# at-wat/mcl_3dl

Hardware: AMD Instinct MI355X
Metric: particle·point evals/sec; filter-update Hz @ 4096 particles × 16k-pt scan (higher is better)
Workload: dtype f32

## Files before the change

### mcl_3dl_amd/csrc/host_map_compilers.h

```cpp
#pragma once

namespace
{
int build_lik_grid(mcl3dl_hip_ctx* ctx);
int build_dda_grid(mcl3dl_hip_ctx* ctx);
int ensure_map_dev(mcl3dl_hip_ctx* ctx);
int cloud_minmax(mcl3dl_hip_ctx* ctx, const float4* pts, long long n, float* host6, unsigned long long* host_cnt);

void kd_ray_radii(const mcl3dl_hip_ctx* ctx, float* grid_min, float* r1, float* r2)
{
  const float mn = std::min({ ctx->map_grid[0], ctx->map_grid[1], ctx->map_grid[2] });
  const float mx = std::max({ ctx->map_grid[0], ctx->map_grid[1], ctx->map_grid[2] });
  *grid_min = mn;
  *r1 = static_cast<float>(std::sqrt(2.0) * mx / 2.0);
  *r2 = static_cast<float>(mn * 2 + std::sqrt(2.0) * mx / 2.0);
}

bool lik_cell_is_beams(const mcl3dl_hip_ctx* ctx)
{
  return !ctx->lik_params_set && ctx->beam_raycast == 1;
}

float lik_cell_edge(const mcl3dl_hip_ctx* ctx)
{
// ... 611 lines not shown
    g.brick_table = table;
    g.rec = ctx->cand_rec.as<float4>();
    g.ovf = ctx->cand_ovf.as<float4>();
    g.ox = cp.ox;
    g.oy = cp.oy;
    g.oz = cp.oz;
    g.inv_ex = cp.inv_ex;
    g.inv_ey = cp.inv_ey;
    g.inv_ez = cp.inv_ez;
    g.nvx = cp.nvx;
    g.nvy = cp.nvy;
    g.nvz = cp.nvz;
    g.nbx = cp.nbx;
    g.nby = cp.nby;
    g.nbz = cp.nbz;
    g.mul24_ok = (static_cast<long long>(cp.nbx) * cp.nby < (1ll << 24) && cp.nbz < (1 << 24)) ? 1 : 0;
    g.off32_ok = (rec_bytes * static_cast<unsigned long long>(n_vox) < (1ull << 32)) ? 1 : 0;
    g.rec_bytes32 = bytes32(rec_bytes * static_cast<unsigned long long>(n_vox));
    g.rec_parts = static_cast<int>(cap);
    set_word_format(g, co.packed, ctx->match_dist_min);
    ctx->cand_parts = cap;
    g.ovf_bytes32 = bytes32(64ull * (n_ovf ? n_ovf : 1));
    g.ti_empty = static_cast<uint32_t>(n_table);
    ctx->footprint[5] = sizeof(int) * n_table;
    ctx->footprint[6] = rec_bytes * static_cast<size_t>(n_vox);
    ctx->footprint[7] = 64ull * n_ovf;
    ctx->cand_stats[0] = n_bricks;
    ctx->cand_stats[1] = static_cast<double>(total);
    ctx->cand_stats[2] = static_cast<double>(kept);
    ctx->cand_stats[3] = ms2;
    ctx->cand_stats[4] = static_cast<double>(co.hist3[0]);
    ctx->cand_stats[5] = static_cast<double>(co.hist3[1]);
    ctx->cand_over8 = static_cast<double>(co.hist3[2]);
    ctx->cand_stats[6] = n_ovf;
    ctx->cand_stats[7] = cp.ex / static_cast<double>(ctx->match_dist_min);
    ctx->cand_edge_ratio[0] = cp.ex / static_cast<double>(ctx->match_dist_min);
    ctx->cand_edge_ratio[1] = cp.ey / static_cast<double>(ctx->match_dist_min);
    ctx->cand_edge_ratio[2] = cp.ez / static_cast<double>(ctx->match_dist_min);
    ctx->cand_dirty = false;
    return 0;
  }
  return ctx->fail(-3, "the candidate index is built for lik_index = 2 only");
}

int build_cand_grid_budgeted(mcl3dl_hip_ctx* ctx, double ratio, uint32_t cap, double* ratio_used = nullptr)
{
// ... 111 lines not shown
  hipLaunchKernelGGL(mc_ovf_counts, dim3(static_cast<unsigned>((n_vox + 1 + 255) / 256)), dim3(256), 0, ctx->stream,
                     ctx->cand_rec.as<float4>(), n_vox, cap, ctx->rg.packed, ctx->rg.count_shift, ctx->rg.count_is_records, cnt);
  TRY(device_exclusive_scan(ctx, cnt, n_vox + 1));
  uint32_t live = 0;
  TRY(d2h(ctx, &live, cnt + n_vox, sizeof(uint32_t)));
  TRY(sync_stream(ctx));
  void* fresh = nullptr;
  const size_t cap_bytes = 64ull * (static_cast<size_t>(live) + live / 2 + 1024);
  HIP_TRY(hipMalloc(&fresh, cap_bytes));
  hipLaunchKernelGGL(mc_ovf_move, dim3(static_cast<unsigned>((n_vox + 255) / 256)), dim3(256), 0, ctx->stream,
                     ctx->cand_rec.as<float4>(), n_vox, cap, ctx->rg.packed, ctx->rg.count_shift, ctx->rg.ext_bits, ctx->rg.count_is_records, cnt,
                     ctx->cand_ovf.as<float4>(),
                     static_cast<float4*>(fresh));
  HIP_TRY(hipGetLastError());
  TRY(sync_stream(ctx));
  if (ctx->cand_ovf.p)
    HIP_TRY(hipFree(ctx->cand_ovf.p));
  ctx->cand_ovf.p = fresh;
  ctx->cand_ovf.cap = cap_bytes;
  ctx->cand_n_ovf = live;
  ctx->cand_ovf_leaked = 0;
  ctx->rg.ovf = ctx->cand_ovf.as<float4>();
  ctx->rg.ovf_bytes32 = bytes32(64ull * (live ? live : 1));
  ctx->footprint[7] = 64ull * live;
  ctx->cand_stats[6] = live;
  ++ctx->cand_ovf_compactions;
  return 0;
}

int update_cand_grid(mcl3dl_hip_ctx* ctx, size_t n_base, const std::vector<float4>& old_update, double* stats5)
{
  const size_t n_total = ctx->map_xyz.size() / 3;
  if (stats5)
    for (int i = 0; i < 6; ++i)
      stats5[i] = 0;
  if (ctx->cand_dirty || ctx->opt.lik_index != 2 || ctx->cand_n_points != n_base + old_update.size())
  {
    if (stats5)
      stats5[5] = ctx->cand_dirty ? 1 : ctx->opt.lik_index != 2 ? 2 : 3;
    ctx->cand_dirty = true;
    return 0;
  }
  CompileParams cp = ctx->cand_cp;
  const long long n_table = ctx->cand_n_table;
  std::vector<float4> fresh;
  TRY(rescaled_points(ctx, n_base, n_total - n_base, fresh, nullptr, nullptr));
// ... 123 lines not shown
  HIP_TRY(hipMemsetAsync(d_orphan.p, 0, sizeof(unsigned long long), ctx->stream));
  hipLaunchKernelGGL(mc_install_records, dim3(static_cast<unsigned>((n_sub_vox + 255) / 256)), dim3(256), 0, ctx->stream,
                     static_cast<const float4*>(d_subrec.p), static_cast<const int*>(d_sub_main.p), ovf_base, n_bricks_old,
                     n_sub_vox, ctx->cand_rec.as<float4>(), static_cast<unsigned long long*>(d_orphan.p), cap, ctx->rg.packed,
                     ctx->rg.count_shift, ctx->rg.count_is_records);
  HIP_TRY(hipGetLastError());
  unsigned long long orphaned = 0;
  TRY(d2h(ctx, &orphaned, d_orphan.p, sizeof(orphaned)));
  HIP_TRY(hipEventRecord(ev1, ctx->stream));
  TRY(sync_stream(ctx));
  float ms = 0.f;
  HIP_TRY(hipEventSynchronize(ev1));
  HIP_TRY(hipEventElapsedTime(&ms, ev0, ev1));
  ctx->cand_n_bricks = n_bricks;
  ctx->cand_n_ovf = ovf_base + co.n_ovf;
  ctx->cand_ovf_leaked += static_cast<uint32_t>(orphaned);
  ctx->cand_n_points = n_total;
  ctx->rg.brick_table = ctx->cand_table.as<int>();
  ctx->rg.rec = ctx->cand_rec.as<float4>();
  ctx->rg.ovf = ctx->cand_ovf.as<float4>();
  ctx->rg.off32_ok = (rec_bytes * 512 * n_bricks < (1ull << 32)) ? 1 : 0;
  ctx->rg.rec_bytes32 = bytes32(rec_bytes * 512 * n_bricks);
  ctx->rg.ovf_bytes32 = bytes32(64ull * (ctx->cand_n_ovf ? ctx->cand_n_ovf : 1));
  ctx->footprint[6] = rec_bytes * 512 * n_bricks;
  ctx->footprint[7] = 64ull * ctx->cand_n_ovf;
  ctx->cand_stats[0] = n_bricks;
  ctx->cand_stats[6] = ctx->cand_n_ovf;
  if (stats5)
  {
    stats5[0] = n_dirty;
    stats5[1] = n_new;
    stats5[2] = n_rel;
    stats5[3] = ms;
    stats5[4] = co.n_ovf;
  }
  return 0;
}

}
```

### mcl_3dl_amd/csrc/host_measure.h

```cpp
#pragma once
#include <type_traits>

namespace
{
int ensure_structures(mcl3dl_hip_ctx* ctx, bool need_lik, bool need_dda, bool need_cells = false)
{
  if (!ctx->has_map)
    return ctx->fail(-5, "no map: call mcl3dl_hip_set_map first");
  bool built = false;
  if (need_lik && ctx->opt.lik_index == 0 && !need_cells && !ctx->lik_params_set && (ctx->lik_cell_from_beam || lik_cell_is_beams(ctx)))
  {
    ctx->lik_params_set = true;
    if (ctx->lik_cell_from_beam)
      ctx->lik_dirty = ctx->lik_base_dirty = true;
  }
  if (need_lik && (ctx->opt.lik_index == 0 || need_cells) && ctx->lik_dirty)
  {
    TRY(build_lik_grid(ctx));
    built = true;
  }
  if (need_lik && ctx->opt.lik_index >= 1 && !need_cells && ctx->cand_dirty)
  {
    TRY(build_cand_grid(ctx));
    built = true;
// ... 211 lines not shown
  long long grid = 0;
};

Interleave interleave(long long n_beam, long long n_other)
{
  Interleave il;
  if (n_beam >= n_other)
    il.beam8 = static_cast<uint32_t>(std::min<long long>(8, (n_beam + n_other / 2) / n_other));
  else
    il.other8 = static_cast<uint32_t>(std::min<long long>(8, (n_other + n_beam / 2) / n_beam));
  const long long rounds = std::max((n_beam + 8 * il.beam8 - 1) / (8 * il.beam8), (n_other + 8 * il.other8 - 1) / (8 * il.other8));
  il.grid = rounds * 8 * (il.beam8 + il.other8);
  return il;
}

bool lik_defer_active(const mcl3dl_hip_ctx* ctx)
{
  if (ctx->opt.lik_defer == 0 || ctx->opt.lik_index != 2 || !ctx->rg.packed || ctx->rg.rec_parts != 4)
    return false;
  if (ctx->opt.lik_defer == 1)
    return true;
  const double with_cand = ctx->cand_stats[4], over4 = ctx->cand_stats[5];
  return with_cand > 0 && over4 / with_cand > LIK_DEFER_MIN_FRAC;
}

int ensure_chain(mcl3dl_hip_ctx* ctx, size_t n_p, int n_tiles, uint32_t* tag0)
{
  if (!ctx->chain_err)
  {
    volatile unsigned* w = ctx->zero_copy_supported ? static_cast<volatile unsigned*>(pinned_alloc(ctx, 64)) : nullptr;
    if (!w || !ctx->zero_copy_supported)
      return ctx->fail(-2, "strict_order = 3 needs page-locked memory the device can write in place");
    *w = 0u;
    ctx->chain_err = w;
  }
  const size_t need = sizeof(unsigned long long) * 2 * n_p;
  const bool fresh = need > ctx->chain_carry.cap;
  TRY(ensure(ctx, ctx->chain_carry, need));
  if (fresh || ctx->chain_tag > 0xffffffffu - static_cast<uint32_t>(n_tiles) - 2u)
  {
    HIP_TRY(hipMemsetAsync(ctx->chain_carry.p, 0, ctx->chain_carry.cap, ctx->stream));
    ctx->chain_tag = 1u;
  }
  *tag0 = ctx->chain_tag;
  ctx->chain_tag += static_cast<uint32_t>(n_tiles) + 1u;
  return 0;
// ... 365 lines not shown
    {
      const auto kernel = ctx->dg.ov_n > 0 ? beam_kernel<false, true> : beam_kernel<false, false>;
      hipLaunchKernelGGL(kernel, grid, dim3(256), 0, bs, c.d_pose, ctx->scan_beam.as<float4>(), static_cast<int>(ctx->n_b),
                         ctx->origins.as<float4>(), pl.n_rays, ctx->dg, beam_params(ctx), ctx->penalty.as<unsigned>(),
                         static_cast<RayStats*>(nullptr), prepared, static_cast<int>(ctx->n_o));
    }
    finish_beam(c, bs);
  }
  TRY(timing_end(ctx, ep, bs));
  if (overlap)
    HIP_TRY(hipEventRecord(ctx->ev_join, bs));
  HIP_TRY(hipGetLastError());
  return 0;
}

template <class Args>
Interleave merged_args(const MeasureCall& c, long long n_beam, long long n_other, Args* a)
{
  mcl3dl_hip_ctx* ctx = c.ctx;
  const Interleave il = interleave(n_beam, n_other);
  a->pose7 = c.d_pose;
  a->n_p = c.np;
  a->g = ctx->lg;
  a->rg = ctx->rg;
  a->prm = c.lp;
  a->scan_beam = ctx->scan_beam.as<float4>();
  a->n_b = static_cast<int>(ctx->n_b);
  a->origins = ctx->origins.as<float4>();
  a->n_rays = c.plan.n_rays;
  a->dg = ctx->dg;
  a->bp = beam_params(ctx);
  a->penalty = ctx->penalty.as<unsigned>();
  a->prepared = c.plan.prepared ? ctx->beam_origin.as<BeamOrigin>() : nullptr;
  a->n_o = static_cast<int>(ctx->n_o);
  a->beam8 = il.beam8;
  a->n_beam_blocks = static_cast<uint32_t>(n_beam);
  return il;
}

template <bool CHAIN>
void launch_lik_beam(const MeasureCall& c, long long t_blocks, const float4* scan, int n_s, int n_tiles, LikBeamArgs& a)
{
  mcl3dl_hip_ctx* ctx = c.ctx;
  const Interleave il = merged_args(c, c.plan.beam_blocks, t_blocks, &a);
  a.n_groups = c.plan.n_groups;
  a.strict_skew4 = STRICT_SKEW4;
  a.tiled8 = il.other8;
// ... 39 lines not shown
}

void launch_tiled(const MeasureCall& c, const float4* t_scan, int t_ns, int t_tiles, double* t_psum, unsigned* t_pcnt,
                  const uint32_t* t_perm, float* t_terms)
{
  mcl3dl_hip_ctx* ctx = c.ctx;
  const MeasurePlan& pl = c.plan;
  const long long t_blocks = tiled_blocks(t_tiles, pl.n_groups);
  if (pl.beam == BeamRoute::MergedTiled)
  {
    LikBeamArgs a{};
    a.partial_sum = t_psum;
    a.partial_cnt = t_pcnt;
    a.scan_perm = t_perm;
    a.strict_terms = t_terms;
    launch_lik_beam<false>(c, t_blocks, t_scan, t_ns, t_tiles, a);
    return;
  }
  dispatch_int<4, 8, 32, 16>(pl.group_size, [&](auto g) {
    dispatch_form(pl, [&](auto mode, auto coop, auto defer) {
      constexpr int G = decltype(g)::value;
      constexpr int MINW = G == 32 ? 4 : 8;
      hipLaunchKernelGGL((likelihood_tiled_kernel<G, decltype(mode)::value, MINW, decltype(coop)::value, decltype(defer)::value>), dim3(static_cast<unsigned>(t_blocks)),
                         dim3(256), 0, ctx->stream, c.d_pose, c.np, t_scan, t_ns, t_tiles, pl.n_groups, ctx->lg, ctx->rg, c.lp,
                         t_psum, t_pcnt, t_perm, t_terms, STRICT_SKEW4);
    });
  });
}

template <int GG>
void launch_strict_sum(mcl3dl_hip_ctx* ctx, const float* strict_terms, int ns, int np, int n_groups, float* d_lik, hipStream_t on,
                       int accumulate)
{
  constexpr int MAX_GPW = 64 / GG >= 4 ? 4 : (64 / GG >= 2 ? 2 : 1);
  int gpw = n_groups <= ctx->n_cus ? 1 : (n_groups <= 2 * ctx->n_cus ? 2 : 4);
  gpw = std::min(gpw, MAX_GPW);
  const auto launch = [&](auto chunk, auto per_wg) {
    constexpr int GPW = decltype(per_wg)::value;
    hipLaunchKernelGGL((lik_strict_sum_rows_kernel<GG, decltype(chunk)::value, GPW>), dim3((n_groups + GPW - 1) / GPW), dim3(1024),
                       0, on, strict_terms, ns, np, n_groups, d_lik, STRICT_SKEW4, accumulate);
  };
  using std::integral_constant;
  if constexpr (MAX_GPW >= 4)
    if (gpw == 4)
      return launch(integral_constant<int, 16384>{}, integral_constant<int, 4>{});
  if constexpr (MAX_GPW >= 2)
    if (gpw >= 2)
      return launch(integral_constant<int, 32768>{}, integral_constant<int, 2>{});
// ... 79 lines not shown
    hipEvent_t ev;
    hipStream_t st;
    ~ChainDone()
    {
      (void)hipEventRecord(ev, st);
    }
  } chain_done{ cs.ev, ctx->stream };
  float* const lik_out = c.d_lik ? c.d_lik : ctx->chain_lik.as<float>();
  const LikChain lc{ ctx->chain_carry.as<unsigned long long>(), pl.chain_tag0, lik_out, c.d_ratio, c.beam_ones(), ctx->chain_err };
  const dim3 grid(static_cast<unsigned>(pl.blocks));
  if (pl.lik == LikRoute::ChainMulti)
    hipLaunchKernelGGL((likelihood_chain_multi_kernel<4, 4>), grid, dim3(256), 0, ctx->stream, c.d_pose, c.np, c.scan, c.ns,
                       pl.n_tiles, pl.n_super, pl.n_groups, ctx->rg, c.lp, lc);
  else if (pl.beam == BeamRoute::MergedChain)
  {
    LikBeamArgs a{};
    a.ch = lc;
    launch_lik_beam<true>(c, pl.blocks, c.scan, c.ns, pl.n_tiles, a);
  }
  else
    dispatch_int<4, 8, 16>(pl.group_size, [&](auto g) {
      dispatch_form(pl, [&](auto mode, auto coop, auto defer) {
        hipLaunchKernelGGL((likelihood_tiled_kernel<decltype(g)::value, decltype(mode)::value, 8, decltype(coop)::value, decltype(defer)::value, true>),
                           grid, dim3(256), 0, ctx->stream, c.d_pose, c.np, c.scan, c.ns, pl.n_tiles, pl.n_groups, ctx->lg, ctx->rg, c.lp,
                           static_cast<double*>(nullptr), static_cast<unsigned*>(nullptr), static_cast<const uint32_t*>(nullptr),
                           static_cast<float*>(nullptr), 0, lc);
      });
    });
  return 0;
}

void launch_particle(const MeasureCall& c)
{
  mcl3dl_hip_ctx* ctx = c.ctx;
  const MeasurePlan& pl = c.plan;
  const uint32_t* row_perm = pl.rows ? ctx->scan_perm.as<uint32_t>() : nullptr;
  const size_t row_bytes = pl.rows ? sizeof(float) * static_cast<size_t>(chain_row_floats(c.ns)) : 0;
  if (pl.beam == BeamRoute::MergedParticle)
  {
    LikParticleBeamArgs a{};
    const Interleave il = merged_args(c, (pl.n_rays + pl.block - 1) / pl.block, c.np, &a);
    a.scan = c.scan;
    a.n_s = c.ns;
    a.out_lik = c.d_lik;
    a.out_ratio = c.d_ratio;
    a.coop = pl.coop ? 1 : 0;
    a.perm = row_perm;
// ... 198 lines not shown
```

### mcl_3dl_amd/csrc/host_options.h

```cpp
#pragma once

#include <cstdio>
#include <cstdlib>
#include <cstring>
#include <limits>

constexpr long long OVERLAP_MIN_RAYS = 262144;
constexpr int LIK_WIDE_MAX_PARTICLES = 512;
constexpr int PF_FUSED_MAX_PARTICLES = 1024;
constexpr int STRICT_ROWS_MAX_PARTICLES = 2048;
constexpr double POLL_QUERY_US = 5000.0;
constexpr double LIK_DEFER_MIN_FRAC = 0.03;
constexpr long long BEAM_PREPARE_MIN_RAYS = 32768;
constexpr int CHAIN_MULTI_MAX = 1536;

struct Options
{
  int overlap_models = 1;
  int lik_index = 2;
  int lik_small = 1;
  int lik_tiled = 1;
  int lik_tiled_min = 1024;
  int lik_group = 0;
  int lik_coop = 1;
  int pf_fused = 1;
  int strict_order = 2;
  int strict_auto_min = 28147;
  int strict_exact_max = 4096;
  double strict_auto_max_bytes = 0.0;
  int strict_chunk = 0;
  int scan_presorted = 0;
  int update_small = 1;
  int update_small_max = 512;
  int update_small_conformant = 0;
  int update_stage = 1;
  int update_zero_copy = 1;
  int poll_sync = 2;
  double poll_spin_us = 2000.0;
  bool test_late_structures = false;
  int cand_prune_coop = 1;
  int batch_slice = 0;
  double cand_voxel_ratio = 0.0;
  double cand_phase = 0.5;
  int cand_aniso = 2;
  double cand_aniso_max = 8.0;
  double index_budget_opt = -1.0;
  int cand_record_parts = 0;
// ... 197 lines not shown
```

### mcl_3dl_amd/csrc/likelihood_kernels.h

```cpp
#pragma once
#include <hip/hip_runtime.h>
#include <stdint.h>

#include "device_math.h"
#include "float_chain.h"
#include "map_structs.h"
#pragma clang fp contract(off)

namespace mcl3dl
{
template <bool STATS>
__device__ inline float nearest_d2(const LikGrid& g, float qx, float qy, float qz, unsigned& n_tested)
{
  const float fx = floorf((qx - g.ox) * g.inv_cell);
  const float fy = floorf((qy - g.oy) * g.inv_cell);
  const float fz = floorf((qz - g.oz) * g.inv_cell);
  float best = 3.0e38f;
  if (!(fx >= 1.0f && fy >= 1.0f && fz >= 1.0f && fx <= static_cast<float>(g.nx - 2) &&
        fy <= static_cast<float>(g.ny - 2) && fz <= static_cast<float>(g.nz - 2)))
    return best;
  const int cx = static_cast<int>(fx), cy = static_cast<int>(fy), cz = static_cast<int>(fz);
  uint32_t rs[9], re[9];
#pragma unroll
  for (int r = 0; r < 9; ++r)
// ... 68 lines not shown
            const float d2 = d2_simple(qx, qy, qz, p.x, p.y, p.z);
            const int idx = static_cast<int>(__float_as_uint(p.w));
            if (d2 < best || (d2 == best && best_idx >= 0 && idx < best_idx))
            {
              best = d2;
              best_idx = idx;
            }
          }
        }
  }
  out_index[i] = best_idx;
  if (out_sqdist)
    out_sqdist[i] = best_idx >= 0 ? best : -1.0f;
}


__device__ inline int floor_to_int(float x)
{
  int r;
  asm("v_cvt_flr_i32_f32 %0, %1" : "=v"(r) : "v"(x));
  return r;
}

__device__ inline bool rec_locate(const RecGrid& g, float qx, float qy, float qz, uint32_t& ti, uint32_t& sub)
{
  const int vx = floor_to_int((qx - g.ox) * g.inv_ex);
  const int vy = floor_to_int((qy - g.oy) * g.inv_ey);
  const int vz = floor_to_int((qz - g.oz) * g.inv_ez);
  if (g.mul24_ok)
    ti = __umul24(static_cast<uint32_t>(vz >> 3), static_cast<uint32_t>(g.nbx * g.nby)) +
         __umul24(static_cast<uint32_t>(vy >> 3), static_cast<uint32_t>(g.nbx)) + static_cast<uint32_t>(vx >> 3);
  else
    ti = (static_cast<uint32_t>(vz >> 3) * static_cast<uint32_t>(g.nby) + static_cast<uint32_t>(vy >> 3)) *
             static_cast<uint32_t>(g.nbx) + static_cast<uint32_t>(vx >> 3);
  sub = ((((static_cast<uint32_t>(vz) & 7u) << 3) | (static_cast<uint32_t>(vy) & 7u)) << 3) | (static_cast<uint32_t>(vx) & 7u);
  return static_cast<unsigned>(vx) < static_cast<unsigned>(g.nvx) && static_cast<unsigned>(vy) < static_cast<unsigned>(g.nvy) &&
         static_cast<unsigned>(vz) < static_cast<unsigned>(g.nvz);
}

__device__ inline float rec_overflow_min(const RecGrid& g, float qx, float qy, float qz, uint32_t n_records, uint32_t ext,
                                         float best)
{
  const float4* o = g.ovf + 4 * static_cast<size_t>(ext);
  for (uint32_t j = 0; j < 4u * n_records; ++j)
  {
    const float4 c = o[j];
    const float d = d2_simple(qx, qy, qz, c.x, c.y, c.z);
    best = d < best ? d : best;
  }
  return best;
}

// ... 53 lines not shown
  return __int_as_float(__builtin_amdgcn_update_dpp(0, __float_as_int(v), CTRL, 0xf, 0xf, true));
}
template <int CTRL>
__device__ inline uint32_t quad_u(uint32_t v)
{
  return static_cast<uint32_t>(__builtin_amdgcn_update_dpp(0, static_cast<int>(v), CTRL, 0xf, 0xf, true));
}
constexpr int QUAD_BCAST0 = 0x00, QUAD_BCAST1 = 0x55, QUAD_BCAST2 = 0xAA, QUAD_BCAST3 = 0xFF;
constexpr int QUAD_XOR1 = 0xB1, QUAD_XOR2 = 0x4E;

typedef unsigned int u32x4 __attribute__((ext_vector_type(4)));
__device__ inline float4 buffer_load_f4(__amdgpu_buffer_rsrc_t rs, uint32_t byte_offset)
{
  const u32x4 v = __builtin_amdgcn_raw_buffer_load_b128(rs, static_cast<int>(byte_offset), 0, 0);
  return make_float4(__uint_as_float(v.x), __uint_as_float(v.y), __uint_as_float(v.z), __uint_as_float(v.w));
}

__device__ inline unsigned long long lanes_gt_u32(uint32_t a, uint32_t b)
{
  return __builtin_amdgcn_uicmp(a, b, 34 );
}
constexpr unsigned long long QUAD_LANE0_MASK = 0x1111111111111111ull;

__device__ inline float quad_round(const float4* recs, uint32_t bytes32, uint32_t rec_index, float qx, float qy, float qz,
                                   int j, uint32_t (&w)[4])
{
  float4 R0, R1, R2, R3;
  if (bytes32)
  {
    const __amdgpu_buffer_rsrc_t rs =
        __builtin_amdgcn_make_buffer_rsrc(const_cast<float4*>(recs), 0, static_cast<int>(bytes32), 0x00020000);
    const uint32_t mine = rec_index << 6, part = static_cast<uint32_t>(j) << 4;
    R0 = buffer_load_f4(rs, quad_u<QUAD_BCAST0>(mine) + part);
    R1 = buffer_load_f4(rs, quad_u<QUAD_BCAST1>(mine) + part);
    R2 = buffer_load_f4(rs, quad_u<QUAD_BCAST2>(mine) + part);
    R3 = buffer_load_f4(rs, quad_u<QUAD_BCAST3>(mine) + part);
  }
  else
  {
    const float4* part = recs + j;
    R0 = part[4 * static_cast<size_t>(quad_u<QUAD_BCAST0>(rec_index))];
    R1 = part[4 * static_cast<size_t>(quad_u<QUAD_BCAST1>(rec_index))];
    R2 = part[4 * static_cast<size_t>(quad_u<QUAD_BCAST2>(rec_index))];
    R3 = part[4 * static_cast<size_t>(quad_u<QUAD_BCAST3>(rec_index))];
  }
  const float d0 = d2_simple(quad_f<QUAD_BCAST0>(qx), quad_f<QUAD_BCAST0>(qy), quad_f<QUAD_BCAST0>(qz), R0.x, R0.y, R0.z);
  const float d1 = d2_simple(quad_f<QUAD_BCAST1>(qx), quad_f<QUAD_BCAST1>(qy), quad_f<QUAD_BCAST1>(qz), R1.x, R1.y, R1.z);
  const float d2 = d2_simple(quad_f<QUAD_BCAST2>(qx), quad_f<QUAD_BCAST2>(qy), quad_f<QUAD_BCAST2>(qz), R2.x, R2.y, R2.z);
  const float d3 = d2_simple(quad_f<QUAD_BCAST3>(qx), quad_f<QUAD_BCAST3>(qy), quad_f<QUAD_BCAST3>(qz), R3.x, R3.y, R3.z);
  const bool odd = (j & 1) != 0, high = (j & 2) != 0;
  const uint32_t u0 = __float_as_uint(d0), u1 = __float_as_uint(d1), u2 = __float_as_uint(d2), u3 = __float_as_uint(d3);
  const uint32_t m01 = min(odd ? u1 : u0, quad_u<QUAD_XOR1>(odd ? u0 : u1));
  const uint32_t m23 = min(odd ? u3 : u2, quad_u<QUAD_XOR1>(odd ? u2 : u3));
  w[0] = __float_as_uint(R0.w);
  w[1] = __float_as_uint(R1.w);
  w[2] = __float_as_uint(R2.w);
  w[3] = __float_as_uint(R3.w);
  return __uint_as_float(min(high ? m23 : m01, quad_u<QUAD_XOR2>(high ? m01 : m23)));
}
// ... 375 lines not shown
  {
    if (out_lik)
      out_lik[p] = lik;
    if (out_ratio)
      out_ratio[p] = static_cast<float>(num) / static_cast<float>(n_s);
  }
}

struct LikChain
{
  unsigned long long* carry;
  uint32_t tag0;
  float* out_lik;
  float* out_ratio;
  float* also_fill;
  volatile unsigned* err;
};

__device__ inline unsigned long long chain_pack(uint32_t value, uint32_t tag)
{
  return (static_cast<unsigned long long>(tag) << 32) | value;
}

constexpr int CHAIN_POLL_MAX = 1 << 20;
constexpr int DEFER_QCAP = 96;

struct DeferQueue
{
  uint32_t word[4][DEFER_QCAP];
  uint16_t who[4][DEFER_QCAP];
};

__device__ inline float eval_coop_first(const RecGrid& rg, const LikParams& prm, const Vec3f pos, const Quat rot, const float4 v,
                                        bool have_point, int lane, bool& matched, bool& over, float& best, uint32_t& mine,
                                        unsigned long long& over_m)
{
  const Vec3f tp = vadd(qrot_trim(rot, Vec3f{ v.x, v.y, v.z }), pos);
  const float qx = tp.x * prm.wx, qy = tp.y * prm.wy, qz = tp.z * prm.wz;
  uint32_t ti, sub;
  const bool inside = rec_locate(rg, qx, qy, qz, ti, sub) && have_point;
  const int b = rg.brick_table[inside ? ti : rg.ti_empty];
  const bool valid = b >= 0;
  float dist = -1.0f;
  over = false;
  over_m = 0ull;
  best = 0.0f;
  mine = 0u;
  const unsigned long long valid_m = __builtin_amdgcn_ballot_w64(valid);
  if (valid_m != 0ull)
  {
    const uint32_t rec = (static_cast<uint32_t>(b) << 9) | sub;
    const uint32_t vrec = rg.rec_bytes32 ? rec : (valid ? rec : 0u);
    uint32_t w[4];
    best = quad_round(rg.rec, rg.rec_bytes32, vrec, qx, qy, qz, lane & 3, w);
    mine = own_word(w, lane & 3);
    over_m = valid_m & lanes_gt_u32(mine, rg.over_thr);
    if (rg.bound_step > 0.0f && over_m != 0ull)
    {
      asm volatile("");
      over_m &= __builtin_amdgcn_fcmpf(best, rec_bound2(rg, mine), 2 );
    }
    over = __builtin_amdgcn_inverse_ballot_w64(over_m);
    if (valid && !over && best < prm.r2)
    {
      const float s = sqrt_in_radius(best);
      dist = lik_dist(prm, s);
    }
  }
  matched = !(dist < 0.0f);
  return lik_term(prm, dist, matched);
}

template <int G, int LD>
__device__ inline void defer_drain(const RecGrid& rg, const LikParams& prm, const float (&s_pose)[G][8], float (&s_term)[G][LD],
                                   unsigned (&s_cnt)[G][4], const DeferQueue& q, int wave, int lane, uint32_t base, uint32_t n,
                                   const float4 v)
{
  const bool act = static_cast<uint32_t>(lane) < n;
  const uint32_t slot = act ? base + static_cast<uint32_t>(lane) : base;
  const uint32_t word = q.word[wave][slot];
  const uint32_t who = q.who[wave][slot];
  const int src = static_cast<int>(who & 63u), k = static_cast<int>(who >> 6);
  const Vec3f pt = { __shfl(v.x, src), __shfl(v.y, src), __shfl(v.z, src) };
  const Vec3f pos = { s_pose[k][0], s_pose[k][1], s_pose[k][2] };
  const Quat rot = { s_pose[k][3], s_pose[k][4], s_pose[k][5], s_pose[k][6] };
  const Vec3f tp = vadd(qrot_trim(rot, pt), pos);
  const float qx = tp.x * prm.wx, qy = tp.y * prm.wy, qz = tp.z * prm.wz;
  const int t_src = wave * 64 + src;
  float best = s_term[k][t_src];
  const uint32_t ext = word & rec_ext_mask(rg);
  const uint32_t rounds = act ? rec_overflow_records(word >> rg.count_shift, 4u, rg.count_is_records) : 0u;
  for (uint32_t r = 0; wave_any(r < rounds); ++r)
  {
    const bool more = r < rounds;
    uint32_t unused[4];
    const float m = quad_round(rg.ovf, rg.ovf_bytes32, more ? ext + r : 0u, qx, qy, qz, lane & 3, unused);
    best = (more && m < best) ? m : best;
  }
  float dist = -1.0f;
  if (act && best < prm.r2)
  {
    const float s = sqrt_in_radius(best);
    dist = lik_dist(prm, s);
  }
  if (act)
  {
    s_term[k][t_src] = lik_term(prm, dist, !(dist < 0.0f));
    if (!(dist < 0.0f))
      atomicAdd(&s_cnt[k][wave], 1u);
  }
}

template <int G, int MODE, int MINW = 8, bool COOP = false, bool DEFER = false, bool CHAIN = false>
__device__ __forceinline__ void likelihood_tiled_body(const uint32_t block_index, const float* __restrict__ pose7, int n_p,
                                                      const float4* __restrict__ scan, int n_s, int n_tiles, int n_groups,
                                                      LikGrid g, RecGrid rg, LikParams prm,
                                                      double* __restrict__ partial_sum, unsigned* __restrict__ partial_cnt,
                                                      const uint32_t* __restrict__ scan_perm, float* __restrict__ strict_terms,
                                                      int strict_skew4, LikChain ch)
{
  constexpr int TERM_LD = CHAIN ? 260 : 256;
  __shared__ float s_pose[G][8];
  __shared__ __attribute__((aligned(16))) float s_term[G][TERM_LD];
  __shared__ unsigned s_cnt[G][4];
  const uint32_t xcd = block_index & 7u;
  const uint32_t seq = block_index >> 3;
  const uint32_t ng = static_cast<uint32_t>(n_groups);
  const uint32_t full_tiles = static_cast<uint32_t>(n_tiles) & ~7u;
  const uint32_t per_xcd_full = (full_tiles >> 3) * ng;
  int tile, group;
  if constexpr (CHAIN)
  {
    const uint32_t row = seq / ng;
    tile = static_cast<int>(row * 8u + xcd);
    group = static_cast<int>(seq - row * ng);
    if (tile >= n_tiles)
      return;
  }
  else if (seq < per_xcd_full)
  {
    const uint32_t row = seq / ng;
    tile = static_cast<int>(row * 8u + xcd);
    group = static_cast<int>(seq - row * ng);
  }
  else
// ... 16 lines not shown
    if (p < n_p)
    {
      const float* ps = pose7 + 7 * static_cast<size_t>(p);
      const Quat r = qnormalized(Quat{ ps[3], ps[4], ps[5], ps[6] });
      s_pose[t][0] = ps[0];
      s_pose[t][1] = ps[1];
      s_pose[t][2] = ps[2];
      s_pose[t][3] = r.x;
      s_pose[t][4] = r.y;
      s_pose[t][5] = r.z;
      s_pose[t][6] = r.w;
      v = 1.f;
    }
    s_pose[t][7] = v;
  }
  const int i = tile * 256 + t;
  const bool have_point = i < n_s;
  const float4 v = have_point ? scan[i] : make_float4(0.f, 0.f, 0.f, 0.f);
  __syncthreads();
  const int n_valid = min(G, n_p - group * G);
  if constexpr (COOP && MODE == 2 && DEFER)
  {
    __shared__ DeferQueue s_q;
    uint32_t qn = 0;
    for (int k = 0; k < n_valid; ++k)
    {
      const Vec3f pos = { s_pose[k][0], s_pose[k][1], s_pose[k][2] };
      const Quat rot = { s_pose[k][3], s_pose[k][4], s_pose[k][5], s_pose[k][6] };
      bool matched, over;
      float best;
      uint32_t mine;
      unsigned long long om;
      const float term = eval_coop_first(rg, prm, pos, rot, v, have_point, lane, matched, over, best, mine, om);
      s_term[k][t] = over ? best : term;
      const unsigned long long m = __builtin_amdgcn_ballot_w64(matched);
      if (lane == 0)
        s_cnt[k][wave] = static_cast<unsigned>(__popcll(m));
      if (om != 0ull)
      {
        const uint32_t n_new = static_cast<uint32_t>(__popcll(om));
        if (qn + n_new > static_cast<uint32_t>(DEFER_QCAP))
        {
          __builtin_amdgcn_fence(__ATOMIC_RELEASE, "wavefront");
          __builtin_amdgcn_wave_barrier();
          defer_drain(rg, prm, s_pose, s_term, s_cnt, s_q, wave, lane, 0u, qn, v);
          qn = 0;
        }
        if (over)
        {
          const uint32_t slot = qn + __builtin_amdgcn_mbcnt_hi(static_cast<uint32_t>(om >> 32),
                                                               __builtin_amdgcn_mbcnt_lo(static_cast<uint32_t>(om), 0u));
          s_q.word[wave][slot] = mine;
          s_q.who[wave][slot] = static_cast<uint16_t>((static_cast<uint32_t>(k) << 6) | static_cast<uint32_t>(lane));
        }
        qn += n_new;
        if (qn >= 64u)
        {
          __builtin_amdgcn_fence(__ATOMIC_RELEASE, "wavefront");
          __builtin_amdgcn_wave_barrier();
          defer_drain(rg, prm, s_pose, s_term, s_cnt, s_q, wave, lane, qn - 64u, 64u, v);
          qn -= 64u;
        }
      }
    }
    if (qn != 0u)
    {
      __builtin_amdgcn_fence(__ATOMIC_RELEASE, "wavefront");
      __builtin_amdgcn_wave_barrier();
      defer_drain(rg, prm, s_pose, s_term, s_cnt, s_q, wave, lane, 0u, qn, v);
    }
  }
  else if constexpr (COOP && MODE == 2)
  {
    for (int k = 0; k < n_valid; ++k)
    {
      const Vec3f pos = { s_pose[k][0], s_pose[k][1], s_pose[k][2] };
      const Quat rot = { s_pose[k][3], s_pose[k][4], s_pose[k][5], s_pose[k][6] };
      bool matched;
      const float term = eval_coop(rg, prm, pos, rot, v, have_point, lane, matched);
      s_term[k][t] = term;
      const unsigned long long m = __builtin_amdgcn_ballot_w64(matched);
      if (lane == 0)
        s_cnt[k][wave] = static_cast<unsigned>(__popcll(m));
    }
  }
  else
  for (int k = 0; k < n_valid; ++k)
  {
    const Vec3f pos = { s_pose[k][0], s_pose[k][1], s_pose[k][2] };
    const Quat rot = { s_pose[k][3], s_pose[k][4], s_pose[k][5], s_pose[k][6] };
    float term = 0.f;
    bool matched = false;
    if (have_point)
// ... 327 lines not shown
```

### mcl_3dl_amd/csrc/map_compiler.h

```cpp
#pragma once
#include <hip/hip_runtime.h>
#include <stdint.h>

namespace mcl3dl
{
struct CompileParams
{
  float ox, oy, oz, inv_ex, inv_ey, inv_ez;
  double ex, ey, ez;
  double grow;
  double r2_hi;
  double margin;
  int rx, ry, rz;
  int nvx, nvy, nvz, nbx, nby, nbz;
  int n_points;
};

__device__ inline int3 voxel_of(const CompileParams& c, const float4 p)
{
  return make_int3(static_cast<int>(floorf((p.x - c.ox) * c.inv_ex)), static_cast<int>(floorf((p.y - c.oy) * c.inv_ey)),
                   static_cast<int>(floorf((p.z - c.oz) * c.inv_ez)));
}

__device__ inline long long brick_index(const CompileParams& c, int vx, int vy, int vz)
// ... 481 lines not shown
        }
        prelim[s + rank] = s_alive[grp][i] ? id : (id | 0x80000000u);
      }
      if (g == 0)
        kept_count[v] = n;
    }
    __syncthreads();
  }
}


constexpr float REC_SENTINEL = 1.0e18f;
constexpr uint32_t REC_EXT_BITS = 26u, REC_EXT_MASK = (1u << REC_EXT_BITS) - 1u, REC_COUNT_MAX = 63u;
constexpr uint32_t REC2_EXT_BITS = 22u, REC2_COUNT_SHIFT = 28u, REC2_BOUND_MAX = 63u;

struct RecGrid
{
  const int32_t* brick_table;
  const float4* rec;
  const float4* ovf;
  float ox, oy, oz, inv_ex, inv_ey, inv_ez;
  int nvx, nvy, nvz, nbx, nby, nbz;
  int mul24_ok;
  int off32_ok;
  uint32_t rec_bytes32, ovf_bytes32;
  int rec_parts;
  uint32_t ti_empty;
  int packed;
  uint32_t count_shift, ext_bits;
  int count_is_records;
  uint32_t over_thr;
  float bound_step;
};

__host__ __device__ inline uint32_t rec_ext_mask(const RecGrid& g)
{
  return (1u << g.ext_bits) - 1u;
}
__host__ __device__ inline uint32_t rec_overflow_records(uint32_t field, uint32_t cap, int count_is_records)
{
  return count_is_records ? field : (field > cap ? (field - cap + 3u) / 4u : 0u);
}
__device__ inline float rec_bound2(const RecGrid& g, uint32_t w)
{
  const float bd = static_cast<float>((w >> REC2_EXT_BITS) & REC2_BOUND_MAX) * g.bound_step;
  return bd * bd;
}

__global__ __launch_bounds__(256) void mc_count_overflow(const uint32_t* __restrict__ kept_count, uint32_t* __restrict__ n_ovf,
                                                         long long n_vox, unsigned long long* __restrict__ hist3, uint32_t cap)
{
  __shared__ unsigned long long s_h[5];
  if (threadIdx.x < 5)
    s_h[threadIdx.x] = 0ull;
  __syncthreads();
  unsigned long long h_any = 0, h_4 = 0, h_8 = 0, h_max = 0, h_15 = 0;
  const long long stride = static_cast<long long>(gridDim.x) * blockDim.x;
// ... 323 lines not shown
```

Measured before the change: 299.3 billion.

## Add specialized fast path for tiled deferred coop likelihood on common map layouts

Adds a runtime-selected FAST template instantiation of the deferred cooperative pose loop. It applies when the map satisfies common conditions: 32-bit offsets, mul24-safe indexing, packed 4-part records, and match distance derived from the radius. The path drops runtime branches for mul24 and buffer-resource selection, and loads the brick table through a raw buffer_load. It also walks LDS pose, term and count pointers incrementally and simplifies the term and match computation using ballots. The cost is inline asm, scheduling barriers and doubled kernel code size. Correctness now depends on the host-side eligibility checks.

```diff
diff --git a/mcl_3dl_amd/csrc/host_map_compilers.h b/mcl_3dl_amd/csrc/host_map_compilers.h
--- a/mcl_3dl_amd/csrc/host_map_compilers.h
+++ b/mcl_3dl_amd/csrc/host_map_compilers.h
@@ -657,6 +657,8 @@
     ctx->cand_parts = cap;
     g.ovf_bytes32 = bytes32(64ull * (n_ovf ? n_ovf : 1));
     g.ti_empty = static_cast<uint32_t>(n_table);
+    g.table_bytes32 = bytes32(sizeof(int) * (static_cast<unsigned long long>(n_table) + 1));
+    g.common_map = rec_common_map(g);
     ctx->footprint[5] = sizeof(int) * n_table;
     ctx->footprint[6] = rec_bytes * static_cast<size_t>(n_vox);
     ctx->footprint[7] = 64ull * n_ovf;
@@ -814,6 +816,7 @@
   ctx->cand_ovf_leaked = 0;
   ctx->rg.ovf = ctx->cand_ovf.as<float4>();
   ctx->rg.ovf_bytes32 = bytes32(64ull * (live ? live : 1));
+  ctx->rg.common_map = rec_common_map(ctx->rg);
   ctx->footprint[7] = 64ull * live;
   ctx->cand_stats[6] = live;
   ++ctx->cand_ovf_compactions;
@@ -983,6 +986,7 @@
   ctx->rg.off32_ok = (rec_bytes * 512 * n_bricks < (1ull << 32)) ? 1 : 0;
   ctx->rg.rec_bytes32 = bytes32(rec_bytes * 512 * n_bricks);
   ctx->rg.ovf_bytes32 = bytes32(64ull * (ctx->cand_n_ovf ? ctx->cand_n_ovf : 1));
+  ctx->rg.common_map = rec_common_map(ctx->rg);
   ctx->footprint[6] = rec_bytes * 512 * n_bricks;
   ctx->footprint[7] = 64ull * ctx->cand_n_ovf;
   ctx->cand_stats[0] = n_bricks;
diff --git a/mcl_3dl_amd/csrc/host_measure.h b/mcl_3dl_amd/csrc/host_measure.h
--- a/mcl_3dl_amd/csrc/host_measure.h
+++ b/mcl_3dl_amd/csrc/host_measure.h
@@ -257,6 +257,19 @@
     return true;
   const double with_cand = ctx->cand_stats[4], over4 = ctx->cand_stats[5];
   return with_cand > 0 && over4 / with_cand > LIK_DEFER_MIN_FRAC;
+}
+
+bool lik_tiled_fast_active(const mcl3dl_hip_ctx* ctx, const LikParams& p)
+{
+  return ctx->opt.lik_tiled_fast != 0 && ctx->rg.common_map && lik_defer_active(ctx) && lik_coop_active(ctx) &&
+         lik_match_from_radius(p.match_dist_min, p.r2, p.match_dist_flat);
+}
+
+RecGrid tiled_rec_grid(const mcl3dl_hip_ctx* ctx, const LikParams& p)
+{
+  RecGrid rg = ctx->rg;
+  rg.common_map = lik_tiled_fast_active(ctx, p) ? 1 : 0;
+  return rg;
 }
 
 int ensure_chain(mcl3dl_hip_ctx* ctx, size_t n_p, int n_tiles, uint32_t* tag0)
@@ -668,7 +681,7 @@
   a->pose7 = c.d_pose;
   a->n_p = c.np;
   a->g = ctx->lg;
-  a->rg = ctx->rg;
+  a->rg = tiled_rec_grid(ctx, c.lp);
   a->prm = c.lp;
   a->scan_beam = ctx->scan_beam.as<float4>();
   a->n_b = static_cast<int>(ctx->n_b);
@@ -754,8 +767,8 @@
       constexpr int G = decltype(g)::value;
       constexpr int MINW = G == 32 ? 4 : 8;
       hipLaunchKernelGGL((likelihood_tiled_kernel<G, decltype(mode)::value, MINW, decltype(coop)::value, decltype(defer)::value>), dim3(static_cast<unsigned>(t_blocks)),
-                         dim3(256), 0, ctx->stream, c.d_pose, c.np, t_scan, t_ns, t_tiles, pl.n_groups, ctx->lg, ctx->rg, c.lp,
-                         t_psum, t_pcnt, t_perm, t_terms, STRICT_SKEW4);
+                         dim3(256), 0, ctx->stream, c.d_pose, c.np, t_scan, t_ns, t_tiles, pl.n_groups, ctx->lg, tiled_rec_grid(ctx, c.lp),
+                         c.lp, t_psum, t_pcnt, t_perm, t_terms, STRICT_SKEW4);
     });
   });
 }
@@ -881,7 +894,8 @@
     dispatch_int<4, 8, 16>(pl.group_size, [&](auto g) {
       dispatch_form(pl, [&](auto mode, auto coop, auto defer) {
         hipLaunchKernelGGL((likelihood_tiled_kernel<decltype(g)::value, decltype(mode)::value, 8, decltype(coop)::value, decltype(defer)::value, true>),
-                           grid, dim3(256), 0, ctx->stream, c.d_pose, c.np, c.scan, c.ns, pl.n_tiles, pl.n_groups, ctx->lg, ctx->rg, c.lp,
+                           grid, dim3(256), 0, ctx->stream, c.d_pose, c.np, c.scan, c.ns, pl.n_tiles, pl.n_groups, ctx->lg,
+                           tiled_rec_grid(ctx, c.lp), c.lp,
                            static_cast<double*>(nullptr), static_cast<unsigned*>(nullptr), static_cast<const uint32_t*>(nullptr),
                            static_cast<float*>(nullptr), 0, lc);
       });
diff --git a/mcl_3dl_amd/csrc/host_options.h b/mcl_3dl_amd/csrc/host_options.h
--- a/mcl_3dl_amd/csrc/host_options.h
+++ b/mcl_3dl_amd/csrc/host_options.h
@@ -1,5 +1,6 @@
 #pragma once
 
+#include <cmath>
 #include <cstdio>
 #include <cstdlib>
 #include <cstring>
@@ -14,6 +15,11 @@
 constexpr long long BEAM_PREPARE_MIN_RAYS = 32768;
 constexpr int CHAIN_MULTI_MAX = 1536;
 
+inline bool lik_match_from_radius(float r, float r2, float flat)
+{
+  return flat <= r && sqrtf(r2) == r;
+}
+
 struct Options
 {
   int overlap_models = 1;
@@ -23,6 +29,7 @@
   int lik_tiled_min = 1024;
   int lik_group = 0;
   int lik_coop = 1;
+  int lik_tiled_fast = -1;
   int pf_fused = 1;
   int strict_order = 2;
   int strict_auto_min = 28147;
diff --git a/mcl_3dl_amd/csrc/likelihood_kernels.h b/mcl_3dl_amd/csrc/likelihood_kernels.h
--- a/mcl_3dl_amd/csrc/likelihood_kernels.h
+++ b/mcl_3dl_amd/csrc/likelihood_kernels.h
@@ -114,12 +114,13 @@
   return r;
 }
 
+template <bool FAST = false>
 __device__ inline bool rec_locate(const RecGrid& g, float qx, float qy, float qz, uint32_t& ti, uint32_t& sub)
 {
   const int vx = floor_to_int((qx - g.ox) * g.inv_ex);
   const int vy = floor_to_int((qy - g.oy) * g.inv_ey);
   const int vz = floor_to_int((qz - g.oz) * g.inv_ez);
-  if (g.mul24_ok)
+  if (FAST || g.mul24_ok)
     ti = __umul24(static_cast<uint32_t>(vz >> 3), static_cast<uint32_t>(g.nbx * g.nby)) +
          __umul24(static_cast<uint32_t>(vy >> 3), static_cast<uint32_t>(g.nbx)) + static_cast<uint32_t>(vx >> 3);
   else
@@ -219,11 +220,12 @@
 }
 constexpr unsigned long long QUAD_LANE0_MASK = 0x1111111111111111ull;
 
+template <bool FAST = false>
 __device__ inline float quad_round(const float4* recs, uint32_t bytes32, uint32_t rec_index, float qx, float qy, float qz,
                                    int j, uint32_t (&w)[4])
 {
   float4 R0, R1, R2, R3;
-  if (bytes32)
+  if (FAST || bytes32)
   {
     const __amdgpu_buffer_rsrc_t rs =
         __builtin_amdgcn_make_buffer_rsrc(const_cast<float4*>(recs), 0, static_cast<int>(bytes32), 0x00020000);
@@ -232,6 +234,8 @@
     R1 = buffer_load_f4(rs, quad_u<QUAD_BCAST1>(mine) + part);
     R2 = buffer_load_f4(rs, quad_u<QUAD_BCAST2>(mine) + part);
     R3 = buffer_load_f4(rs, quad_u<QUAD_BCAST3>(mine) + part);
+    if constexpr (FAST)
+      __builtin_amdgcn_sched_barrier(0);
   }
   else
   {
@@ -653,6 +657,12 @@
   return (static_cast<unsigned long long>(tag) << 32) | value;
 }
 
+template <bool B>
+struct BoolConstant
+{
+  static constexpr bool value = B;
+};
+
 constexpr int CHAIN_POLL_MAX = 1 << 20;
 constexpr int DEFER_QCAP = 96;
 
@@ -662,15 +672,25 @@
   uint16_t who[4][DEFER_QCAP];
 };
 
+template <bool FAST = false>
 __device__ inline float eval_coop_first(const RecGrid& rg, const LikParams& prm, const Vec3f pos, const Quat rot, const float4 v,
                                         bool have_point, int lane, bool& matched, bool& over, float& best, uint32_t& mine,
-                                        unsigned long long& over_m)
+                                        unsigned long long& over_m, unsigned long long* matched_m = nullptr)
 {
   const Vec3f tp = vadd(qrot_trim(rot, Vec3f{ v.x, v.y, v.z }), pos);
   const float qx = tp.x * prm.wx, qy = tp.y * prm.wy, qz = tp.z * prm.wz;
   uint32_t ti, sub;
-  const bool inside = rec_locate(rg, qx, qy, qz, ti, sub) && have_point;
-  const int b = rg.brick_table[inside ? ti : rg.ti_empty];
+  const bool inside = rec_locate<FAST>(rg, qx, qy, qz, ti, sub) && have_point;
+  int b;
+  if constexpr (FAST)
+  {
+    const unsigned long long base = reinterpret_cast<unsigned long long>(rg.brick_table);
+    const u32x4 tb = { static_cast<uint32_t>(base), (static_cast<uint32_t>(base >> 32) & 0xffffu) | (4u << 16), rg.table_bytes32,
+                       0x00020000u };
+    asm volatile("buffer_load_dword %0, %1, %2, 0 idxen\n\ts_waitcnt vmcnt(0)" : "=v"(b) : "v"(inside ? ti : rg.ti_empty), "s"(tb) : "memory");
+  }
+  else
+    b = rg.brick_table[inside ? ti : rg.ti_empty];
   const bool valid = b >= 0;
   float dist = -1.0f;
   over = false;
@@ -680,10 +700,14 @@
   const unsigned long long valid_m = __builtin_amdgcn_ballot_w64(valid);
   if (valid_m != 0ull)
   {
-    const uint32_t rec = (static_cast<uint32_t>(b) << 9) | sub;
-    const uint32_t vrec = rg.rec_bytes32 ? rec : (valid ? rec : 0u);
+    if constexpr (FAST)
+      asm("" : "+v"(sub));
+    uint32_t rec = (static_cast<uint32_t>(b) << 9) | sub;
+    if constexpr (FAST)
+      asm("" : "+v"(rec));
+    const uint32_t vrec = (FAST || rg.rec_bytes32) ? rec : (valid ? rec : 0u);
     uint32_t w[4];
-    best = quad_round(rg.rec, rg.rec_bytes32, vrec, qx, qy, qz, lane & 3, w);
+    best = quad_round<FAST>(rg.rec, rg.rec_bytes32, vrec, qx, qy, qz, lane & 3, w);
     mine = own_word(w, lane & 3);
     over_m = valid_m & lanes_gt_u32(mine, rg.over_thr);
     if (rg.bound_step > 0.0f && over_m != 0ull)
@@ -692,17 +716,33 @@
       over_m &= __builtin_amdgcn_fcmpf(best, rec_bound2(rg, mine), 2 );
     }
     over = __builtin_amdgcn_inverse_ballot_w64(over_m);
+    if constexpr (FAST)
+    {
+      const unsigned long long in_m = valid_m & ~over_m & __builtin_amdgcn_fcmpf(best, prm.r2, 4 );
+      float out = over ? best : 0.0f * prm.match_weight;
+      if (__builtin_amdgcn_inverse_ballot_w64(in_m))
+        out = lik_dist(prm, sqrt_in_radius(best)) * prm.match_weight;
+      *matched_m = in_m;
+      matched = __builtin_amdgcn_inverse_ballot_w64(in_m);
+      return out;
+    }
     if (valid && !over && best < prm.r2)
     {
       const float s = sqrt_in_radius(best);
       dist = lik_dist(prm, s);
     }
   }
+  if constexpr (FAST)
+  {
+    *matched_m = 0ull;
+    matched = false;
+    return 0.0f * prm.match_weight;
+  }
   matched = !(dist < 0.0f);
   return lik_term(prm, dist, matched);
 }
 
-template <int G, int LD>
+template <bool FAST = false, int G, int LD>
 __device__ inline void defer_drain(const RecGrid& rg, const LikParams& prm, const float (&s_pose)[G][8], float (&s_term)[G][LD],
                                    unsigned (&s_cnt)[G][4], const DeferQueue& q, int wave, int lane, uint32_t base, uint32_t n,
                                    const float4 v)
@@ -725,8 +765,19 @@
   {
     const bool more = r < rounds;
     uint32_t unused[4];
-    const float m = quad_round(rg.ovf, rg.ovf_bytes32, more ? ext + r : 0u, qx, qy, qz, lane & 3, unused);
+    const float m = quad_round<FAST>(rg.ovf, rg.ovf_bytes32, more ? ext + r : 0u, qx, qy, qz, lane & 3, unused);
     best = (more && m < best) ? m : best;
+  }
+  if constexpr (FAST)
+  {
+    if (act)
+    {
+      const bool in = best < prm.r2;
+      s_term[k][t_src] = in ? lik_dist(prm, sqrt_in_radius(best)) * prm.match_weight : 0.0f * prm.match_weight;
+      if (in)
+        atomicAdd(&s_cnt[k][wave], 1u);
+    }
+    return;
   }
   float dist = -1.0f;
   if (act && best < prm.r2)
@@ -751,7 +802,7 @@
                                                       int strict_skew4, LikChain ch)
 {
   constexpr int TERM_LD = CHAIN ? 260 : 256;
-  __shared__ float s_pose[G][8];
+  __shared__ __attribute__((aligned(16))) float s_pose[G][8];
   __shared__ __attribute__((aligned(16))) float s_term[G][TERM_LD];
   __shared__ unsigned s_cnt[G][4];
   const uint32_t xcd = block_index & 7u;
@@ -814,53 +865,83 @@
   if constexpr (COOP && MODE == 2 && DEFER)
   {
     __shared__ DeferQueue s_q;
-    uint32_t qn = 0;
-    for (int k = 0; k < n_valid; ++k)
-    {
-      const Vec3f pos = { s_pose[k][0], s_pose[k][1], s_pose[k][2] };
-      const Quat rot = { s_pose[k][3], s_pose[k][4], s_pose[k][5], s_pose[k][6] };
-      bool matched, over;
-      float best;
-      uint32_t mine;
-      unsigned long long om;
-      const float term = eval_coop_first(rg, prm, pos, rot, v, have_point, lane, matched, over, best, mine, om);
-      s_term[k][t] = over ? best : term;
-      const unsigned long long m = __builtin_amdgcn_ballot_w64(matched);
-      if (lane == 0)
-        s_cnt[k][wave] = static_cast<unsigned>(__popcll(m));
-      if (om != 0ull)
+    const auto pose_loop = [&](auto fast) {
+      constexpr bool FAST = decltype(fast)::value;
+      uint32_t qn = 0;
+      typedef float f32x4 __attribute__((ext_vector_type(4)));
+      typedef __attribute__((address_space(3))) const f32x4 LdsPose;
+      typedef __attribute__((address_space(3))) float LdsTerm;
+      typedef __attribute__((address_space(3))) unsigned LdsCount;
+      LdsPose* p_pose = (LdsPose*)&s_pose[0][0];
+      LdsTerm* p_term = (LdsTerm*)&s_term[0][t];
+      LdsCount* p_cnt = (LdsCount*)&s_cnt[0][wave];
+      for (int k = 0; k < n_valid; ++k)
       {
-        const uint32_t n_new = static_cast<uint32_t>(__popcll(om));
-        if (qn + n_new > static_cast<uint32_t>(DEFER_QCAP))
+        LdsPose* ps = FAST ? p_pose : (LdsPose*)&s_pose[k][0];
+        const f32x4 pa = ps[0], pb = ps[1];
+        const Vec3f pos = { pa.x, pa.y, pa.z };
+        const Quat rot = { pa.w, pb.x, pb.y, pb.z };
+        bool matched, over;
+        float best;
+        uint32_t mine;
+        unsigned long long om;
+        unsigned long long m;
+        if constexpr (FAST)
         {
-          __builtin_amdgcn_fence(__ATOMIC_RELEASE, "wavefront");
-          __builtin_amdgcn_wave_barrier();
-          defer_drain(rg, prm, s_pose, s_term, s_cnt, s_q, wave, lane, 0u, qn, v);
-          qn = 0;
+          *p_term = eval_coop_first<true>(rg, prm, pos, rot, v, have_point, lane, matched, over, best, mine, om, &m);
+          if (lane == 0)
+            *p_cnt = static_cast<unsigned>(__popcll(m));
+          asm volatile("" : "+v"(p_pose), "+v"(p_term), "+v"(p_cnt));
+          p_pose += 2;
+          p_term += TERM_LD;
+          p_cnt += 4;
         }
-        if (over)
+        else
         {
-          const uint32_t slot = qn + __builtin_amdgcn_mbcnt_hi(static_cast<uint32_t>(om >> 32),
-                                                               __builtin_amdgcn_mbcnt_lo(static_cast<uint32_t>(om), 0u));
-          s_q.word[wave][slot] = mine;
-          s_q.who[wave][slot] = static_cast<uint16_t>((static_cast<uint32_t>(k) << 6) | static_cast<uint32_t>(lane));
+          const float term = eval_coop_first(rg, prm, pos, rot, v, have_point, lane, matched, over, best, mine, om);
+          s_term[k][t] = over ? best : term;
+          m = __builtin_amdgcn_ballot_w64(matched);
+          if (lane == 0)
+            s_cnt[k][wave] = static_cast<unsigned>(__popcll(m));
         }
-        qn += n_new;
-        if (qn >= 64u)
+        if (om != 0ull)
         {
-          __builtin_amdgcn_fence(__ATOMIC_RELEASE, "wavefront");
-          __builtin_amdgcn_wave_barrier();
-          defer_drain(rg, prm, s_pose, s_term, s_cnt, s_q, wave, lane, qn - 64u, 64u, v);
-          qn -= 64u;
+          const uint32_t n_new = static_cast<uint32_t>(__popcll(om));
+          if (qn + n_new > static_cast<uint32_t>(DEFER_QCAP))
+          {
+            __builtin_amdgcn_fence(__ATOMIC_RELEASE, "wavefront");
+            __builtin_amdgcn_wave_barrier();
+            defer_drain<FAST>(rg, prm, s_pose, s_term, s_cnt, s_q, wave, lane, 0u, qn, v);
+            qn = 0;
+          }
+          if (over)
+          {
+            const uint32_t slot = qn + __builtin_amdgcn_mbcnt_hi(static_cast<uint32_t>(om >> 32),
+                                                                 __builtin_amdgcn_mbcnt_lo(static_cast<uint32_t>(om), 0u));
+            s_q.word[wave][slot] = mine;
+            s_q.who[wave][slot] = static_cast<uint16_t>((static_cast<uint32_t>(k) << 6) | static_cast<uint32_t>(lane));
+          }
+          qn += n_new;
+          if (qn >= 64u)
+          {
+            __builtin_amdgcn_fence(__ATOMIC_RELEASE, "wavefront");
+            __builtin_amdgcn_wave_barrier();
+            defer_drain<FAST>(rg, prm, s_pose, s_term, s_cnt, s_q, wave, lane, qn - 64u, 64u, v);
+            qn -= 64u;
+          }
         }
       }
-    }
-    if (qn != 0u)
-    {
-      __builtin_amdgcn_fence(__ATOMIC_RELEASE, "wavefront");
-      __builtin_amdgcn_wave_barrier();
-      defer_drain(rg, prm, s_pose, s_term, s_cnt, s_q, wave, lane, 0u, qn, v);
-    }
+      if (qn != 0u)
+      {
+        __builtin_amdgcn_fence(__ATOMIC_RELEASE, "wavefront");
+        __builtin_amdgcn_wave_barrier();
+        defer_drain<FAST>(rg, prm, s_pose, s_term, s_cnt, s_q, wave, lane, 0u, qn, v);
+      }
+    };
+    if (rg.common_map)
+      pose_loop(BoolConstant<true>{});
+    else
+      pose_loop(BoolConstant<false>{});
   }
   else if constexpr (COOP && MODE == 2)
   {
diff --git a/mcl_3dl_amd/csrc/map_compiler.h b/mcl_3dl_amd/csrc/map_compiler.h
--- a/mcl_3dl_amd/csrc/map_compiler.h
+++ b/mcl_3dl_amd/csrc/map_compiler.h
@@ -527,6 +527,8 @@
   float ox, oy, oz, inv_ex, inv_ey, inv_ez;
   int nvx, nvy, nvz, nbx, nby, nbz;
   int mul24_ok;
+  int common_map;
+  uint32_t table_bytes32;
   int off32_ok;
   uint32_t rec_bytes32, ovf_bytes32;
   int rec_parts;
@@ -538,6 +540,10 @@
   float bound_step;
 };
 
+__host__ __device__ inline int rec_common_map(const RecGrid& g)
+{
+  return (g.rec_bytes32 != 0u && g.ovf_bytes32 != 0u && g.table_bytes32 != 0u && g.mul24_ok && g.packed && g.rec_parts == 4) ? 1 : 0;
+}
 __host__ __device__ inline uint32_t rec_ext_mask(const RecGrid& g)
 {
   return (1u << g.ext_bits) - 1u;
```

After: 305.0 billion (median of 6 runs). 1.02x the previous value.
